# reedrosenbluth/LASS

Measured on AMD Instinct MI355X. Metric: clips/sec (10s@16kHz), higher is better.
Workload: dtype f32; 1 GPU; ResUNet30 separate() fp32, batch=16/GPU, 10s@16kHz clips, fixed precomputed condition embedding, seeded random-init weights (BASELINE configs[1]); samples_per_clip=160000, parallelism=clip-sharded x1

## Files before the change

### __graft_entry__.py

```python
import os
import subprocess
import sys

ROOT = os.path.dirname(os.path.abspath(__file__))
CSRC = os.path.join(ROOT, "lass_amd", "csrc")
LIB = os.path.join(CSRC, "liblass_hip.so")
SOURCES = ["api.hip", "conv.hip", "wino.hip", "wino4.hip", "pw_gemm.hip", "conv_bf16.hip", "conv_bf16_fused.hip", "stft.hip", "misc.hip", "text.hip", "audio_clap.hip", "resample.hip"]
FLAGS = ["-O3", "-std=c++17", "--offload-arch=gfx950", "-fPIC", "-fno-slp-vectorize"]
EXTRA_FLAGS = {}


def _hipcc() -> str:
    for c in (os.environ.get("HIPCC"), "/opt/rocm/bin/hipcc", "hipcc"):
        if c and (os.path.isabs(c) and os.path.exists(c) or not os.path.isabs(c)):
            return c
    return "hipcc"


STAMP = LIB + ".srchash"


def _src_hash() -> str:
    import hashlib

    h = hashlib.sha256()
    import glob

    h.update(repr((FLAGS, sorted(EXTRA_FLAGS.items()))).encode())

    deps = [os.path.join(CSRC, s) for s in SOURCES] + sorted(glob.glob(os.path.join(CSRC, "*.h"))) + [os.path.join(ROOT, "include", "lass_hip.h")]
    for d in deps:
        h.update(os.path.basename(d).encode())
        with open(d, "rb") as f:
            h.update(f.read())
    return h.hexdigest()


def _stale() -> bool:
    if not os.path.exists(LIB) or not os.path.exists(STAMP):
        return True
    with open(STAMP) as f:
        return f.read().strip() != _src_hash()


def build(force: bool = False) -> None:
    import fcntl

    if force or _stale():
        with open(os.path.join(CSRC, ".build.lock"), "w") as lock:
            fcntl.flock(lock, fcntl.LOCK_EX)
            if force or _stale():
                tmp = LIB + f".tmp{os.getpid()}"
                flags = FLAGS
                objs = [os.path.join(CSRC, f".{os.getpid()}.{s}.o") for s in SOURCES]
                print("[build]", _hipcc(), " ".join(flags), "-c", " ".join(SOURCES), "(parallel) && link", file=sys.stderr, flush=True)
                try:
                    procs = [subprocess.Popen([_hipcc()] + flags + EXTRA_FLAGS.get(s, []) + ["-c", s, "-o", o], cwd=CSRC)
                             for s, o in zip(SOURCES, objs)]
                    rcs = [pr.wait() for pr in procs]
                    if any(rcs):
# ... 54 lines not shown
```

### include/lass_hip.h

```cpp
#ifndef LASS_HIP_H
#define LASS_HIP_H

#include <stddef.h>
#include <stdint.h>

#ifdef __cplusplus
extern "C" {
#endif

typedef struct lass_ctx lass_ctx;

#define LASS_OK 0
#define LASS_ERR_ARG (-1)
#define LASS_ERR_HIP (-2)
#define LASS_ERR_STATE (-3)
#define LASS_ERR_WORKSPACE (-4)

#define LASS_F32 0
#define LASS_I64 1

#define LASS_COMPUTE_F32 0
#define LASS_COMPUTE_BF16 1
#define LASS_COMPUTE_BF16X3 2

int lass_version(void);

int lass_create(lass_ctx** out, int device_id);
int lass_create_multistft(lass_ctx** out, int device_id, int n_fft, int n_windows, const int* win_lengths,
                          int mask_window);
int lass_destroy(lass_ctx* ctx);

const char* lass_last_error(const lass_ctx* ctx);

int lass_set_param(lass_ctx* ctx, const char* name, const void* data, const int64_t* shape, int ndim, int dtype);

int lass_finalize(lass_ctx* ctx, int compute_mode);

int lass_workspace_bytes(const lass_ctx* ctx, int B, int L, size_t* bytes);

int lass_separate(lass_ctx* ctx, const float* mixture, const float* condition, float* out, int B, int L,
                  void* workspace, size_t workspace_bytes, void* stream);

int lass_graph_stats(const lass_ctx* ctx, long* captures, long* replays);
int lass_set_graph_replay(lass_ctx* ctx, int enabled);
int lass_set_wino4_splits(lass_ctx* ctx, int splits);

int lass_separate_components(lass_ctx* ctx, const float* const* mag, const float* cos_mask, const float* sin_mask,
                             const float* condition, float* out, int B, int L, void* workspace, size_t workspace_bytes,
                             void* stream);


int lass_stft_magphase(lass_ctx* ctx, const float* wav, int B, int L, float* mag, float* cos_out, float* sin_out,
                       float* real_out, float* imag_out, void* stream);

int lass_multi_stft(lass_ctx* ctx, const float* wav, int B, int L, int hop, int n_windows, const int* win_lengths,
                    float* const* mag, float* const* cos_out, float* const* sin_out, void* stream);

int lass_stft_components(lass_ctx* ctx, const float* wav, int B, int L, int n_fft, int hop, int n_windows,
                         const int* win_lengths, float* const* mag, float* const* cos_out, float* const* sin_out,
                         void* stream);

int lass_istft(lass_ctx* ctx, const float* real, const float* imag, int B, int T, int L, float* wav,
               float* frames_ws, void* stream);
int lass_istft_nfft(lass_ctx* ctx, const float* real, const float* imag, int B, int T, int L, int n_fft, int win_length,
                    float* wav, void* stream);

int lass_film(lass_ctx* ctx, const float* condition, int B, float* shift, void* stream);
int lass_film_width(const lass_ctx* ctx);
int lass_film_offset(const lass_ctx* ctx, const char* site);
int lass_film_raw(lass_ctx* ctx, const float* condition, int B, float* film, void* stream);

int lass_convblock(lass_ctx* ctx, const char* prefix, const float* x, int B, int H, int W, const float* shift,
                   float* y, float* scratch, void* stream);

int lass_encoder_block(lass_ctx* ctx, const char* name, const float* x, int B, int H, int W, const float* shift, float* y,
                       float* pool, float* scratch, void* stream);

int lass_front_end(lass_ctx* ctx, const float* wav, int B, int L, float* mag, float* cos_out, float* sin_out, float* x0,
                   void* stream);

int lass_workspace_tensor(const lass_ctx* ctx, int B, int L, const char* name, size_t* offset, int64_t shape[4],
                          int64_t strides[4]);

int lass_upconv(lass_ctx* ctx, const char* name, const float* x, int B, int h, int w, const float* shift, float* y,
                void* stream);

int lass_mask_apply(lass_ctx* ctx, const float* x12, const float* mag, const float* cos_in, const float* sin_in,
                    int B, int T, int Tpad, float* out_real, float* out_imag, void* stream);

int lass_sdr_stats(lass_ctx* ctx, const float* ref, const float* est, int B, int L, double* stats, void* stream);

int lass_mix_at_snr(lass_ctx* ctx, float* source, const float* noise, const float* snr_db, float* mixture, int B, int L,
                    double* scratch, void* stream);

#define LASS_WAV_PCM16 0
#define LASS_WAV_PCM32 1
#define LASS_WAV_F32 2
#define LASS_RESAMPLE_MAX_TAPS 16383
// ... 55 lines not shown
```

### lass_amd/_lib.py

```python
from __future__ import annotations

import ctypes
import os
from ctypes import POINTER, c_char_p, c_double, c_int, c_int64, c_long, c_size_t, c_void_p

_HERE = os.path.dirname(os.path.abspath(__file__))
LIB_PATH = os.environ.get("LASS_HIP_LIB") or os.path.join(_HERE, "csrc", "liblass_hip.so")

_lib = None

SYMBOLS = [
    ("lass_version", c_int, []),
    ("lass_create", c_int, [POINTER(c_void_p), c_int]),
    ("lass_create_multistft", c_int, [POINTER(c_void_p), c_int, c_int, c_int, POINTER(c_int), c_int]),
    ("lass_destroy", c_int, [c_void_p]),
    ("lass_last_error", c_char_p, [c_void_p]),
    ("lass_set_param", c_int, [c_void_p, c_char_p, c_void_p, POINTER(c_int64), c_int, c_int]),
    ("lass_finalize", c_int, [c_void_p, c_int]),
    ("lass_workspace_bytes", c_int, [c_void_p, c_int, c_int, POINTER(c_size_t)]),
    ("lass_separate", c_int, [c_void_p, c_void_p, c_void_p, c_void_p, c_int, c_int, c_void_p, c_size_t, c_void_p]),
    ("lass_stft_magphase", c_int, [c_void_p, c_void_p, c_int, c_int, c_void_p, c_void_p, c_void_p, c_void_p,
                                   c_void_p, c_void_p]),
    ("lass_mix_at_snr", c_int, [c_void_p, c_void_p, c_void_p, c_void_p, c_void_p, c_int, c_int, c_void_p, c_void_p]),
    ("lass_decode_resample", c_int, [c_void_p, c_void_p, c_int64, c_int, c_int, c_int, c_int, c_int, c_int, c_void_p, c_int,
                                     c_void_p, c_int, c_void_p]),
    ("lass_segment_mix", c_int, [c_void_p, c_void_p, c_int, c_int, c_void_p, c_void_p, c_int, c_void_p, c_void_p, c_void_p,
                                 c_void_p, c_void_p]),
    ("lass_multi_stft", c_int, [c_void_p, c_void_p, c_int, c_int, c_int, c_int, POINTER(c_int), POINTER(c_void_p),
                                POINTER(c_void_p), POINTER(c_void_p), c_void_p]),
    ("lass_graph_stats", c_int, [c_void_p, POINTER(c_long), POINTER(c_long)]),
    ("lass_set_graph_replay", c_int, [c_void_p, c_int]),
    ("lass_set_wino4_splits", c_int, [c_void_p, c_int]),
    ("lass_separate_components", c_int, [c_void_p, POINTER(c_void_p), c_void_p, c_void_p, c_void_p, c_void_p, c_int,
                                         c_int, c_void_p, c_size_t, c_void_p]),
    ("lass_stft_components", c_int, [c_void_p, c_void_p, c_int, c_int, c_int, c_int, c_int, POINTER(c_int),
                                     POINTER(c_void_p), POINTER(c_void_p), POINTER(c_void_p), c_void_p]),
    ("lass_istft_nfft", c_int, [c_void_p, c_void_p, c_void_p, c_int, c_int, c_int, c_int, c_int, c_void_p, c_void_p]),
    ("lass_istft", c_int, [c_void_p, c_void_p, c_void_p, c_int, c_int, c_int, c_void_p, c_void_p, c_void_p]),
    ("lass_film", c_int, [c_void_p, c_void_p, c_int, c_void_p, c_void_p]),
    ("lass_film_width", c_int, [c_void_p]),
    ("lass_film_offset", c_int, [c_void_p, c_char_p]),
    ("lass_film_raw", c_int, [c_void_p, c_void_p, c_int, c_void_p, c_void_p]),
    ("lass_convblock", c_int, [c_void_p, c_char_p, c_void_p, c_int, c_int, c_int, c_void_p, c_void_p, c_void_p,
                               c_void_p]),
    ("lass_encoder_block", c_int, [c_void_p, c_char_p, c_void_p, c_int, c_int, c_int, c_void_p, c_void_p, c_void_p,
                                   c_void_p, c_void_p]),
    ("lass_front_end", c_int, [c_void_p, c_void_p, c_int, c_int, c_void_p, c_void_p, c_void_p, c_void_p, c_void_p]),
    ("lass_workspace_tensor", c_int, [c_void_p, c_int, c_int, c_char_p, POINTER(c_size_t), POINTER(c_int64),
                                      POINTER(c_int64)]),
    ("lass_upconv", c_int, [c_void_p, c_char_p, c_void_p, c_int, c_int, c_int, c_void_p, c_void_p, c_void_p]),
    ("lass_mask_apply", c_int, [c_void_p, c_void_p, c_void_p, c_void_p, c_void_p, c_int, c_int, c_int, c_void_p,
                                c_void_p, c_void_p]),
    ("lass_sdr_stats", c_int, [c_void_p, c_void_p, c_void_p, c_int, c_int, c_void_p, c_void_p]),
    ("lass_text_create", c_int, [POINTER(c_void_p), c_int]),
    ("lass_text_destroy", c_int, [c_void_p]),
    ("lass_text_last_error", c_char_p, [c_void_p]),
    ("lass_text_set_param", c_int, [c_void_p, c_char_p, c_void_p, POINTER(c_int64), c_int]),
    ("lass_text_finalize", c_int, [c_void_p]),
    ("lass_text_layers", c_int, [c_void_p]),
    ("lass_text_workspace_bytes", c_int, [c_void_p, c_int, c_int, POINTER(c_size_t)]),
    ("lass_text_encode", c_int, [c_void_p, c_void_p, c_void_p, c_int, c_int, c_void_p, c_void_p, c_void_p, c_size_t,
                                 c_void_p]),
    ("lass_audioq_create", c_int, [POINTER(c_void_p), c_int]),
    ("lass_audioq_destroy", c_int, [c_void_p]),
    ("lass_audioq_last_error", c_char_p, [c_void_p]),
    ("lass_audioq_set_param", c_int, [c_void_p, c_char_p, c_void_p, POINTER(c_int64), c_int]),
    ("lass_audioq_finalize", c_int, [c_void_p]),
    ("lass_audioq_stages", c_int, [c_void_p]),
    ("lass_audioq_workspace_bytes", c_int, [c_void_p, c_int, POINTER(c_size_t)]),
    ("lass_audioq_encode_wave48k", c_int, [c_void_p, c_void_p, POINTER(c_int), c_int, c_int, c_void_p, c_void_p, c_void_p,
                                           c_size_t, c_void_p]),
    ("lass_audioq_encode_wave32k", c_int, [c_void_p, c_void_p, POINTER(c_int), c_int, c_int, c_void_p, c_void_p, c_void_p,
                                           c_size_t, c_void_p]),
    ("lass_set_profiling", c_int, [c_void_p, c_int]),
    ("lass_profile_count", c_int, [c_void_p]),
    ("lass_profile_get", c_int, [c_void_p, c_int, POINTER(c_char_p), POINTER(c_double), POINTER(c_int)]),
    ("lass_profile_reset", c_int, [c_void_p]),
]


class LassError(RuntimeError):
    pass


def load():
# ... 24 lines not shown
```

### lass_amd/csrc/api.hip

```cpp
#include <hip/hip_runtime.h>

#include <algorithm>
#include <cmath>
#include <cstdio>
#include <cstdlib>
#include <cstring>
#include <map>
#include <string>
#include <vector>

#include "../../include/lass_hip.h"
#include "kernels.h"

namespace {

struct EncSpec { const char* name; int cin, cout, dh, dw; };
struct DecSpec { const char* name; int cin, cout, uh, uw; };
const EncSpec kEnc[7] = {{"encoder_block1", 32, 32, 2, 2},   {"encoder_block2", 32, 64, 2, 2},
                         {"encoder_block3", 64, 128, 2, 2},  {"encoder_block4", 128, 256, 2, 2},
                         {"encoder_block5", 256, 384, 2, 2}, {"encoder_block6", 384, 384, 1, 2},
                         {"conv_block7a", 384, 384, 1, 1}};
const DecSpec kDec[6] = {{"decoder_block1", 384, 384, 1, 2}, {"decoder_block2", 384, 384, 2, 2},
                         {"decoder_block3", 384, 256, 2, 2}, {"decoder_block4", 256, 128, 2, 2},
                         {"decoder_block5", 128, 64, 2, 2},  {"decoder_block6", 64, 32, 2, 2}};
// ... 20 lines not shown
    int width = 0;
    int s1 = -1, s2 = -1;
    float *w1 = nullptr, *w2 = nullptr, *wsc = nullptr;
    float *u1 = nullptr, *u2 = nullptr, *usc = nullptr;
    float *u1f = nullptr, *u2f = nullptr;
    void *b1 = nullptr, *b2 = nullptr, *bsc16 = nullptr;
    void *b1l = nullptr, *b2l = nullptr, *bscl = nullptr;
    const float* bsc = nullptr;
};

struct ProfEntry {
    const char* name;
    double ms = 0;
    int launches = 0;
};

thread_local std::string g_create_err;

}

struct Geometry {
    int variant = 0;
    int nbr = 1;
    int wins[kMaxBranches] = {1024, 0, 0, 0};
    int nfft = 1024, nbins = 513, fcrop = 512;
    int mask_br = 0;
    int magphase_sem = 0;
};

struct lass_ctx {
    int device = 0;
    std::string err;
    Geometry g;
    EncSpec E[7];
    DecSpec D[6];
    int dec_cat[6] = {0};
    std::string pre_name[kMaxBranches];
    std::map<std::string, Raw> raw;
    bool finalized = false;
    float2* tw2k = nullptr;
    std::vector<Site> sites;
    std::map<std::string, int> site_idx;
    int n_shift = 0;
    float *film_W = nullptr, *film_b = nullptr, *bn_scale = nullptr, *bn_base = nullptr;
    float *bn0_s = nullptr, *bn0_h = nullptr;
    std::vector<ResBlock> enc, dec;
    int dec_site[6] = {0};
    void* up16[6] = {nullptr};
    void* up16l[6] = {nullptr};
    std::vector<void*> owned;
    int compute_mode = LASS_COMPUTE_F32;
    int wino4_mincin = 32;
    int ksplit_force = 0;
    float* stage_part = nullptr;
    size_t stage_part_floats = 0;
    bool fuse_catb = true;
    bool fuse_block = true;
    bool fuse_up = true;
    void* up_sc16 = nullptr;
    bool use_graph = true;
    struct GraphKey {
        const void *mix = nullptr, *cond = nullptr, *out = nullptr, *ws = nullptr;
        int B = 0, L = 0;
        unsigned long gen = 0;
        bool operator==(const GraphKey& o) const {
            return mix == o.mix && cond == o.cond && out == o.out && ws == o.ws && B == o.B && L == o.L && gen == o.gen;
        }
    };
    struct GraphEntry {
        GraphKey key;
        hipGraphExec_t exec = nullptr;
        size_t need = 0;
        int seen = 0;
        unsigned long used = 0;
        bool split = false;
    };
    std::map<std::pair<int, int>, bool> last_split;
    static constexpr int kGraphSlots = 4;
    GraphEntry g_slots[kGraphSlots];
    unsigned long g_tick = 0;
    std::vector<hipGraphExec_t> g_retired;
    hipStream_t g_stream = nullptr;
    int split_batch = 1;
    hipStream_t s2 = nullptr;
    hipEvent_t ev_fork = nullptr, ev_join = nullptr;
    unsigned long gen = 0;
    long g_replays = 0, g_captures = 0;
    bool profiling = false;
    std::vector<ProfEntry> prof;
    std::vector<hipEvent_t> ev_pool;
    struct Pending { int cls; hipEvent_t a, b; };
    std::vector<Pending> pending;
    size_t ev_used = 0;
};

namespace {

#define HIP_TRY(ctx, expr)                                                                                     \
    do {                                                                                                       \
        hipError_t _e = (expr);                                                                                \
        if (_e != hipSuccess) {                                                                                \
            (ctx)->err = std::string(#expr) + ": " + hipGetErrorString(_e);                                     \
            return LASS_ERR_HIP;                                                                               \
        }                                                                                                      \
    } while (0)

// ... 374 lines not shown
            return fail(c, LASS_ERR_STATE, "decoder_block6 with its transposed conv inside needs the fused bf16 kernel");
        ProfScope ps(c, st, P_CONV3X3);
        HIP_TRY(c, lass_launch_dec6u_fused_bf16(p, q, uq, st));
        return 0;
    }
    if (bf2 && !x0 && c->fuse_block && c->compute_mode == LASS_COMPUTE_BF16 && cat_in && f.head && rb.cin != rb.cout &&
        lass_dec6_fused_bf16_supported(p, q)) {
        ProfScope ps(c, st, P_CONV3X3);
        HIP_TRY(c, lass_launch_dec6_fused_bf16(p, q, st));
        return 0;
    }
    const bool sc_gemm = c->compute_mode == LASS_COMPUTE_F32 && !bf2 && rb.cin != rb.cout && !f.head && rb.cin >= kShortcutGemmMinCin &&
                         wino2 && q.w_wino4 && (ksplit > 0 || lass_wino4_supported(CONV2_SHORTCUT, q)) && lass_pw_gemm_supported(CONV2_SHORTCUT, q);
    if (sc_gemm) {
        const auto overlaps = [&](const float* a, long a_bs, long a_n, const float* b, long b_bs, long b_n) {
            return a < b + (size_t)(B - 1) * b_bs + b_n && b < a + (size_t)(B - 1) * a_bs + a_n;
        };
        if (overlaps(out, out_bs, rb.cout * HW, x, x_bs, rb.cin * HW) || overlaps(out, out_bs, rb.cout * HW, a2, rb.cout * HW, rb.cout * HW))
            return fail(c, LASS_ERR_STATE, "a block's output must not overlap its input or its intermediate");
        ProfScope ps(c, st, P_CONV3X3);
        HIP_TRY(c, lass_launch_pw_gemm(CONV2_SHORTCUT, q, st));
    }
    if (int r1 = launch_conv1()) return r1;
    ProfScope ps(c, st, P_CONV3X3);
    if (sc_gemm) {
        ConvArgs r = q;
        r.in2 = nullptr; r.in2_bs = 0; r.Cin2 = 0; r.w2 = nullptr; r.bias = nullptr;
        r.res = out; r.res_bs = out_bs;
        if (!lass_wino4_supported(CONV2_IDENT, r, sk)) return fail(c, LASS_ERR_STATE, "conv2 with the shortcut as residual");
        HIP_TRY(c, lass_launch_wino4(CONV2_IDENT, r, st, sk));
    } else if (rb.cin == rb.cout) {
        if (bf2)
            HIP_TRY(c, lass_launch_conv_bf16(k2, q, st));
        else if (wino2 && (x0 || ksplit > 0) && q.w_wino4 && lass_wino4_supported(k2, q, sk))
            HIP_TRY(c, lass_launch_wino4(k2, q, st, sk));
        else if (wino2)
            HIP_TRY(c, lass_launch_wino(k2, q, st));
        else
            HIP_TRY(c, lass_launch_conv(k2, q, st));
    } else {
        if (bf2)
            HIP_TRY(c, lass_launch_conv_bf16(CONV2_SHORTCUT, q, st));
        else if (wino2 && q.w_wino4 && lass_wino4_supported(CONV2_SHORTCUT, q))
            HIP_TRY(c, lass_launch_wino4(CONV2_SHORTCUT, q, st));
        else if (wino2)
            HIP_TRY(c, lass_launch_wino(CONV2_SHORTCUT, q, st));
        else
            HIP_TRY(c, lass_launch_conv(CONV2_SHORTCUT, q, st));
    }
    return 0;
}

constexpr int kTconvGemmMinCin = 128;

int run_upconv(lass_ctx* c, int di, const float* x, int B, int h, int w, const float* shift, float* out, long out_bs,
               hipStream_t st, const CatCopies* cb = nullptr, bool x_is_act_bf16 = false) {
    const DecSpec& d = c->D[di];
    const Site& s = c->sites[c->dec_site[di]];
    ConvArgs p;
    p.in = x; p.in_bs = (long)d.cin * h * w; p.Cin = d.cin;
    p.w = rawp(c, std::string("base.") + d.name + ".conv1.weight");
    p.N = p.Nw = d.cout * d.uh * d.uw;
    p.pro_scale = c->bn_scale + s.off; p.pro_shift = shift + s.off; p.pro_shift_bs = c->n_shift;
    p.out = out; p.out_bs = out_bs; p.B = B; p.H = h; p.W = w; p.up_h = d.uh;
    p.w_bf16 = c->up16[di]; p.w_bf16_lo = c->up16l[di];
    if (x_is_act_bf16) {
        if (c->compute_mode != LASS_COMPUTE_BF16 || !p.w_bf16 || !lass_bf16_supported(p))
            return fail(c, LASS_ERR_STATE, "activated bf16 input needs the bf16 kernels");
        p.in_bf16 = x;
    }
    if (cb) {
        if (c->compute_mode != LASS_COMPUTE_BF16 || !p.w_bf16 || !lass_bf16_supported(p))
            return fail(c, LASS_ERR_STATE, "blocked bf16 concat copies need the bf16 kernels");
        p.out = nullptr;
        p.out_bf16 = cb->raw; p.out_bf16_act = cb->act; p.out_oct0 = 0; p.out_noct = cb->noct;
        p.act_scale = cb->scale; p.act_shift = cb->shift; p.act_shift_bs = c->n_shift;
    }
    ProfScope ps(c, st, P_TCONV);
    if (c->compute_mode != LASS_COMPUTE_F32 && p.w_bf16 && lass_bf16_supported(p))
        HIP_TRY(c, lass_launch_conv_bf16(TCONV_ACT, p, st));
    else if (c->compute_mode == LASS_COMPUTE_F32 && d.cin >= kTconvGemmMinCin && lass_pw_gemm_supported(TCONV_ACT, p))
        HIP_TRY(c, lass_launch_pw_gemm(TCONV_ACT, p, st));
    else
        HIP_TRY(c, lass_launch_conv(TCONV_ACT, p, st));
    return 0;
}

struct Plan {
    int B, L, T, Tp;
    size_t total = 0;
    size_t mag, cosv, sinv, x0[kMaxBranches], shift, a2, cat[6], pool[6], center, decout[6], oreal, oimag;
    size_t kpart = 0;
    bool has_kpart = false;
    int eh[7], ew[7];
};

size_t bump(size_t& total, size_t floats) {
    const size_t off = total;
    total += (floats * sizeof(float) + 255) / 256 * 256;
    return off;
}

int make_plan(const lass_ctx* c, int B, int L, Plan* pl) {
    const Geometry& g = c->g;
    if (B <= 0 || L <= g.nfft / 2) return LASS_ERR_ARG;
    pl->B = B; pl->L = L;
    pl->T = 1 + L / LASS_HOP;
    pl->Tp = (pl->T + 31) / 32 * 32;
    const size_t clip_max = (size_t)c->dec_cat[5] * pl->Tp * g.fcrop * sizeof(float);
    if (clip_max > 0xFFFF0000ull) return LASS_ERR_ARG;
    size_t& t = pl->total;
    t = 0;
    const size_t spec = (size_t)B * pl->T * g.nbins;
    pl->mag = bump(t, spec); pl->cosv = bump(t, spec); pl->sinv = bump(t, spec);
    for (int k = 0; k < g.nbr; ++k) pl->x0[k] = bump(t, (size_t)B * pl->Tp * g.fcrop);
    pl->shift = bump(t, (size_t)B * c->n_shift);
    int h = pl->Tp, w = g.fcrop;
    size_t a2max = 0;
    for (int i = 0; i < 7; ++i) {
        pl->eh[i] = h; pl->ew[i] = w;
        const size_t o = (size_t)B * c->E[i].cout * h * w;
        if (o > a2max) a2max = o;
        h /= c->E[i].dh; w /= c->E[i].dw;
        if (i < 6) pl->pool[i] = bump(t, (size_t)B * c->E[i].cout * (i == 0 ? g.nbr : 1) * h * w);
    }
    pl->center = bump(t, (size_t)B * c->E[6].cout * pl->eh[6] * pl->ew[6]);
    for (int d = 0; d < 6; ++d) {
        const int e = 5 - d;
        const size_t hw = (size_t)pl->eh[e] * pl->ew[e];
        pl->cat[d] = bump(t, (size_t)B * c->dec_cat[d] * hw);
        pl->decout[d] = bump(t, (size_t)B * c->D[d].cout * hw);
    }
    pl->a2 = bump(t, a2max);
    pl->oreal = bump(t, spec); pl->oimag = bump(t, spec);
    size_t kmax = 0;
    for (int i = 1; i < 7; ++i) {
        const ResBlock& rb = trunk_block(c, i);
// ... 866 lines not shown
                if (r0) return r0;
                Plan pl0;
                if (!condition || !out || !workspace || make_plan(c, B, L, &pl0) || workspace_bytes < pl0.total ||
                    ((uintptr_t)workspace & 255) != 0)
                    return separate_any(c, mixture, condition, out, B, L, workspace, workspace_bytes, (hipStream_t)stream, false);
                slot->need = pl0.total;
                if (split_halves(c, B)) {
                    Plan ph0;
                    if (!make_plan(c, B / 2, L, &ph0) && 2 * ((ph0.total + 255) / 256 * 256) <= workspace_bytes)
                        slot->need = std::max(slot->need, 2 * ((ph0.total + 255) / 256 * 256));
                }
            }
            HIP_TRY(c, hipSetDevice(c->device));
            if (!c->g_stream) HIP_TRY(c, hipStreamCreateWithFlags(&c->g_stream, hipStreamNonBlocking));
            bool ok = false;
            if (hipStreamBeginCapture(c->g_stream, hipStreamCaptureModeThreadLocal) == hipSuccess) {
                const int r = separate_any(c, mixture, condition, out, B, L, workspace, workspace_bytes, c->g_stream, true);
                hipGraph_t graph = nullptr;
                const hipError_t e = hipStreamEndCapture(c->g_stream, &graph);
                if (r == 0 && e == hipSuccess && graph && hipGraphInstantiate(&slot->exec, graph, nullptr, nullptr, 0) == hipSuccess) {
                    ok = true;
                    if (auto it = c->last_split.find({B, L}); it != c->last_split.end()) slot->split = it->second;
                } else {
                    slot->exec = nullptr;
                }
                if (graph) (void)hipGraphDestroy(graph);
            }
            if (ok) {
                ++c->g_captures;
                HIP_TRY(c, hipGraphLaunch(slot->exec, (hipStream_t)stream));
                return 0;
            }
            (void)hipGetLastError();
            c->use_graph = false;
            c->err.clear();
        }
    }
    return separate_any(c, mixture, condition, out, B, L, workspace, workspace_bytes, (hipStream_t)stream, false);
}

int lass_set_graph_replay(lass_ctx* c, int enabled) {
    if (!c) return LASS_ERR_ARG;
    c->use_graph = enabled != 0;
    return 0;
}

int lass_set_wino4_splits(lass_ctx* c, int splits) {
    if (!c || (splits != 0 && splits != 1 && splits != 2 && splits != 4)) return fail(c, LASS_ERR_ARG, "lass_set_wino4_splits: 0, 1, 2 or 4");
    c->ksplit_force = splits;
    ++c->gen;
    return 0;
}

int lass_graph_stats(const lass_ctx* c, long* captures, long* replays) {
    if (!c) return LASS_ERR_ARG;
    if (captures) *captures = c->g_captures;
    if (replays) *replays = c->g_replays;
    return c->use_graph ? 1 : 0;
}

int lass_separate_components(lass_ctx* c, const float* const* mag, const float* cos_mask, const float* sin_mask,
                             const float* condition, float* out, int B, int L, void* workspace, size_t workspace_bytes,
                             void* stream) {
    if (!c) return LASS_ERR_ARG;
    if (!mag || !cos_mask || !sin_mask) return fail(c, LASS_ERR_ARG, "lass_separate_components: null pointer");
    Components comp;
    for (int k = 0; k < kMaxBranches; ++k) comp.mag[k] = k < c->g.nbr ? mag[k] : nullptr;
    comp.cosv = cos_mask; comp.sinv = sin_mask;
    return separate_impl(c, nullptr, &comp, condition, out, B, L, workspace, workspace_bytes, stream,
                         "lass_separate_components");
}

int lass_set_profiling(lass_ctx* c, int enabled) {
    if (!c) return LASS_ERR_ARG;
    if (enabled && c->ev_pool.size() < 2 * kProfPairs) {
        HIP_TRY(c, hipSetDevice(c->device));
        c->pending.reserve(kProfPairs);
        while (c->ev_pool.size() < 2 * kProfPairs) {
            hipEvent_t e;
            HIP_TRY(c, hipEventCreate(&e));
            c->ev_pool.push_back(e);
        }
    }
    c->profiling = enabled != 0;
    return 0;
}
int lass_profile_count(const lass_ctx* c) { return c ? P_COUNT : LASS_ERR_ARG; }
int lass_profile_get(lass_ctx* c, int i, const char** name, double* ms, int* launches) {
    if (!c || i < 0 || i >= P_COUNT) return LASS_ERR_ARG;
    prof_collect(c);
    if (name) *name = c->prof[i].name;
    if (ms) *ms = c->prof[i].ms;
    if (launches) *launches = c->prof[i].launches;
    return 0;
}
int lass_profile_reset(lass_ctx* c) {
    if (!c) return LASS_ERR_ARG;
    prof_collect(c);
    for (auto& p : c->prof) { p.ms = 0; p.launches = 0; }
    return 0;
}

}
```

### lass_amd/csrc/kernels.h

```cpp
#pragma once
#include <hip/hip_runtime.h>
#include <stddef.h>
#include <stdint.h>

constexpr int LASS_NFFT = 1024;
constexpr int LASS_HOP = 160;
constexpr int LASS_NBINS = 513;
constexpr int LASS_FCROP = 512;
constexpr int LASS_COND = 512;
constexpr int LASS_MAX_STFT_WINDOWS = 4;

struct ConvArgs {
    const float* in = nullptr;
    long in_bs = 0;
    int Cin = 0;
    const float* w = nullptr;
    int Nw = 0;
    const float* pro_scale = nullptr;
    const float* pro_shift = nullptr;
    int pro_shift_bs = 0;
    const float* in2 = nullptr;
    long in2_bs = 0;
    int Cin2 = 0;
    const float* w2 = nullptr;
// ... 22 lines not shown
    void* out_bf16_act = nullptr;
    const float* act_scale = nullptr;
    const float* act_shift = nullptr;
    int act_shift_bs = 0;
    int out_oct0 = 0;
    int out_noct = 0;
    const void* in2_bf16 = nullptr;
    void* pool_bf16 = nullptr;
    void* pool_bf16_act = nullptr;
    int pool_oct0 = 0;
    int pool_noct = 0;
    const float* pool_act_scale = nullptr;
    const float* pool_act_shift = nullptr;
    const float* pre_w = nullptr;
    const float* pre_b = nullptr;
    const float* mask_w = nullptr;
    const float* mask_b = nullptr;
    const float* mask_mag = nullptr;
    const float* mask_cos = nullptr;
    const float* mask_sin = nullptr;
    float* mask_re = nullptr;
    float* mask_im = nullptr;
    int mask_T = 0;
    int mask_nbins = LASS_NBINS;
    float* pool_out = nullptr;
    long pool_bs = 0;
    int pool_h = 2;
    int gx = 0, gy = 0;
    int xcd_map = 0;
};

inline bool lass_wino4_narrow(int H, int W) { return W % 32 == 16 && H % 32 == 0; }
struct Wino4Split {
    int n = 1;
    float* part = nullptr;
};

enum ConvKind { CONV1_ACT = 0, CONV2_IDENT = 1, CONV2_SHORTCUT = 2, TCONV_ACT = 3, CONV1_ACT_PRE = 4, CONV2_IDENT_PRE = 5 };

hipError_t lass_launch_conv(ConvKind kind, const ConvArgs& p, hipStream_t stream);

bool lass_wino_supported(const ConvArgs& p);
hipError_t lass_launch_wino(ConvKind kind, const ConvArgs& p, hipStream_t stream);
hipError_t lass_launch_wino_weights(const float* w, int Cout, int Cin, float* U, hipStream_t stream);
hipError_t lass_launch_wino_shortcut_weights(const float* w, int Cout, int Cin, float* U, hipStream_t stream);

bool lass_wino4_supported(ConvKind kind, const ConvArgs& p, const Wino4Split& sk = Wino4Split());
hipError_t lass_launch_wino4(ConvKind kind, const ConvArgs& p, hipStream_t stream, const Wino4Split& sk = Wino4Split());
hipError_t lass_launch_wino4_weights(const float* w, int Cout, int Cin, float* U, hipStream_t stream);

bool lass_pw_gemm_supported(ConvKind kind, const ConvArgs& p);
hipError_t lass_launch_pw_gemm(ConvKind kind, const ConvArgs& p, hipStream_t stream);

bool lass_bf16_supported(const ConvArgs& p);
hipError_t lass_launch_conv_bf16(ConvKind kind, const ConvArgs& p, hipStream_t stream);
hipError_t lass_launch_weights_bf16(const float* w, int Cout, int Cin, int taps, void* dst, int lo, int transposed,
                                    hipStream_t stream);

bool lass_enc1_fused_bf16_supported(const ConvArgs& p, const ConvArgs& q);
hipError_t lass_launch_enc1_fused_bf16(const ConvArgs& p, const ConvArgs& q, hipStream_t stream);
bool lass_dec6_fused_bf16_supported(const ConvArgs& p, const ConvArgs& q);
hipError_t lass_launch_dec6_fused_bf16(const ConvArgs& p, const ConvArgs& q, hipStream_t stream);

bool lass_dec6u_fused_bf16_supported(const ConvArgs& p, const ConvArgs& q, const ConvArgs& u);
hipError_t lass_launch_dec6u_fused_bf16(const ConvArgs& p, const ConvArgs& q, const ConvArgs& u, hipStream_t stream);
hipError_t lass_launch_compose_up_shortcut(const float* wsc, const float* wt, int Cin, int Cup, int Ccat, int Nsc, float* out,
                                           hipStream_t stream);

hipError_t lass_launch_multi_stft(const float* wav, int B, int L, int hop, int nwin, const int* n_fft,
                                  const float2* tw2k, float* const* mag, float* const* cosv, float* const* sinv,
                                  hipStream_t stream);
struct StftBranch {
    int wlen = 0;
    float *mag = nullptr, *cosv = nullptr, *sinv = nullptr, *real = nullptr, *imag = nullptr, *x0 = nullptr;
};
hipError_t lass_launch_stft2(const float* wav, int B, int L, int n_fft, int hop, int T, int Tpad, int nbr,
                             const StftBranch* br, int magphase_sem, const float* s0, const float* h0,
                             const float2* tw2k, hipStream_t stream);
hipError_t lass_launch_istft2(const float* real, const float* imag, int B, int T, int L, int n_fft, int wlen, int hop,
                              const float2* tw2k, float* wav, hipStream_t stream);

hipError_t lass_launch_film(const float* cond, int B, const float* Wf, const float* bf, const float* base, int n,
                            float* out, hipStream_t stream);
hipError_t lass_launch_pool(const float* in, long in_bs, int B, int C, int H, int W, int ph, int pw, float* out,
                            hipStream_t stream);
hipError_t lass_launch_mask(const float* x12, const float* wa, const float* ba, const float* mag, const float* cosv,
                            const float* sinv, int B, int T, int Tpad, int fcrop, float* out_real, float* out_imag,
                            hipStream_t stream);
hipError_t lass_launch_x0_from_mag(const float* mag, int B, int T, int Tpad, int fcrop, const float* s0,
                                   const float* h0, float* x0, hipStream_t stream);
hipError_t lass_launch_sdr(const float* ref, const float* est, int B, int L, double* stats, hipStream_t stream);
hipError_t lass_launch_mix_at_snr(float* source, const float* noise, const float* snr_db, float* mixture, int B, int L,
                                  double* ws, hipStream_t stream);
hipError_t lass_launch_segment_mix(const float* waveforms, int B, int L, const int* mix_num, const float* comp_db, int max_comp,
                                   const float* noise_db, float* mixture, float* segment, double* ws, hipStream_t stream);
hipError_t lass_launch_relayout_conv(const float* src, int Cout, int Cin, int taps, float* dst, hipStream_t stream);
hipError_t lass_launch_bnfold(const float* g, const float* beta, const float* mean, const float* var, int C, float eps,
                              float* scale, float* base, hipStream_t stream);

size_t lass_resample_table_floats(int up, int n_taps);
hipError_t lass_launch_decode_resample(const void* raw, long long row_stride, int B, int frames, int ch, int enc, int up, int down,
                                       const float* taps, int n_taps, float* out, int L_out, hipStream_t stream);
```

### lass_amd/engine.py

```python
from __future__ import annotations

from ctypes import byref, c_char_p, c_double, c_int, c_int64, c_size_t, c_void_p
from typing import Dict, Optional

import numpy as np
import torch

from . import _lib, arch


def _ptr(t: Optional[torch.Tensor]):
    return c_void_p(t.data_ptr()) if t is not None else c_void_p(0)


def _stream(device) -> c_void_p:
    return c_void_p(torch.cuda.current_stream(device).cuda_stream)


class Engine:

    def __init__(self, device="cuda:0", multistft=None):
        self.lib = _lib.load()
        self.device = torch.device(device)
        if self.device.type != "cuda":
# ... 297 lines not shown
            raise _lib.LassError(f"encoding must be one of {sorted(rs.ENCODINGS)}")
        B = raw_u8.shape[0]
        if raw_u8.shape[1] < int(frames) * int(channels) * rs.SAMPLE_BYTES[encoding]:
            raise _lib.LassError("raw_u8 rows are shorter than frames x channels samples")
        up, down = rs.ratio(rate_in, rate_out)
        L_out = rs.out_len(frames, up, down)
        fir = (up, down) != (1, 1)
        if fir and not rs.within_cap(up, down):
            raise _lib.LassError(f"resampling {rate_in} -> {rate_out} Hz needs {rs.n_taps(up, down)} taps, over the device "
                                 f"kernel's cap of {rs.MAX_TAPS}: resample on the host (wavio.read_wav)")
        taps = rs.device_taps(up, down, self.device) if fir else None
        if out is None:
            out = torch.empty(B, L_out, dtype=torch.float32, device=self.device)
        elif (tuple(out.shape) != (B, L_out) or out.dtype != torch.float32 or out.device != self.device
              or not out.is_contiguous()):
            raise _lib.LassError(f"out must be a contiguous float32 {(B, L_out)} tensor on {self.device}")
        stride = raw_u8.stride(0) if B > 1 else (raw_u8.shape[1] + 3) // 4 * 4
        rc = self.lib.lass_decode_resample(self.ctx, _ptr(raw_u8), stride, B, int(frames), int(channels), rs.ENCODINGS[encoding], up, down, _ptr(taps),
                                           taps.numel() if fir else 1, _ptr(out), L_out, _stream(self.device))
        _lib.check(self.ctx, rc, "lass_decode_resample")
        return out

    def resample(self, x: torch.Tensor, rate_in: int, rate_out: int) -> torch.Tensor:
        x = self._dev(x)
        one = x.dim() == 1
        x = x[None] if one else x
        y = self.decode_resample(x.view(torch.uint8), x.shape[1], 1, "f32", rate_in, rate_out)
        return y[0] if one else y

    def segment_mix(self, waveforms: torch.Tensor, mix_num: torch.Tensor, comp_db: torch.Tensor, noise_db: torch.Tensor):
        waveforms = self._dev(waveforms)
        B, L = waveforms.shape
        mix_num = mix_num.to(device=self.device, dtype=torch.int32).contiguous()
        comp_db = comp_db.to(device=self.device, dtype=torch.float32).contiguous()
        noise_db = noise_db.to(device=self.device, dtype=torch.float32).contiguous()
        if mix_num.shape != (B,) or noise_db.shape != (B,) or comp_db.dim() != 2 or comp_db.shape[0] != B:
            raise ValueError("segment_mix: mix_num (B), comp_db (B, max_mix_num - 1), noise_db (B) expected")
        mixture, segment = torch.empty_like(waveforms), torch.empty_like(waveforms)
        scratch = torch.empty(B, 4, dtype=torch.float64, device=self.device)
        rc = self.lib.lass_segment_mix(self.ctx, _ptr(waveforms), B, L, _ptr(mix_num), _ptr(comp_db), int(comp_db.shape[1]),
                                       _ptr(noise_db), _ptr(mixture), _ptr(segment), _ptr(scratch), _stream(self.device))
        _lib.check(self.ctx, rc, "lass_segment_mix")
        return mixture, segment

    def graph_stats(self):
        from ctypes import c_long
        cap, rep = c_long(), c_long()
        on = self.lib.lass_graph_stats(self.ctx, byref(cap), byref(rep))
        return bool(on), cap.value, rep.value

    def set_graph_replay(self, on: bool):
        _lib.check(self.ctx, self.lib.lass_set_graph_replay(self.ctx, 1 if on else 0), "lass_set_graph_replay")

    def set_profiling(self, on: bool):
        self.lib.lass_set_profiling(self.ctx, 1 if on else 0)

    def profile(self, reset: bool = True) -> Dict[str, tuple]:
        out = {}
        for i in range(self.lib.lass_profile_count(self.ctx)):
            name, ms, n = c_char_p(), c_double(), c_int()
            self.lib.lass_profile_get(self.ctx, i, byref(name), byref(ms), byref(n))
            out[name.value.decode()] = (ms.value, n.value)
        if reset:
            self.lib.lass_profile_reset(self.ctx)
        return out


def arch_cond() -> int:
    return 512


_ENGINES: Dict[int, Engine] = {}


def get_engine(device) -> Engine:
    device = torch.device(device)
    idx = device.index if device.index is not None else torch.cuda.current_device()
    if idx not in _ENGINES:
        _ENGINES[idx] = Engine(torch.device("cuda", idx))
    return _ENGINES[idx]
```

Measured before the change: 1040 clips/s.

## Add persistent streaming MFMA kernel for small-Cin transposed convolutions

Adds a persistent-workgroup fp32 MFMA kernel for decoder transposed convolutions with Cin 64 or 128. The weights stay resident in LDS, the fused BN+leaky prologue is applied while staging input chunks, and global loads of the next chunk and next tile are software-pipelined. It is routed by default in f32 mode ahead of the previous pw_gemm and direct paths. The cost is extra LDS pressure and a grid tied to the CU count, which may limit occupancy.

```diff
diff --git a/__graft_entry__.py b/__graft_entry__.py
--- a/__graft_entry__.py
+++ b/__graft_entry__.py
@@ -5,7 +5,7 @@
 ROOT = os.path.dirname(os.path.abspath(__file__))
 CSRC = os.path.join(ROOT, "lass_amd", "csrc")
 LIB = os.path.join(CSRC, "liblass_hip.so")
-SOURCES = ["api.hip", "conv.hip", "wino.hip", "wino4.hip", "pw_gemm.hip", "conv_bf16.hip", "conv_bf16_fused.hip", "stft.hip", "misc.hip", "text.hip", "audio_clap.hip", "resample.hip"]
+SOURCES = ["api.hip", "conv.hip", "wino.hip", "wino4.hip", "pw_gemm.hip", "tconv_stream.hip", "conv_bf16.hip", "conv_bf16_fused.hip", "stft.hip", "misc.hip", "text.hip", "audio_clap.hip", "resample.hip"]
 FLAGS = ["-O3", "-std=c++17", "--offload-arch=gfx950", "-fPIC", "-fno-slp-vectorize"]
 EXTRA_FLAGS = {}
 
diff --git a/include/lass_hip.h b/include/lass_hip.h
--- a/include/lass_hip.h
+++ b/include/lass_hip.h
@@ -44,6 +44,9 @@
 int lass_graph_stats(const lass_ctx* ctx, long* captures, long* replays);
 int lass_set_graph_replay(lass_ctx* ctx, int enabled);
 int lass_set_wino4_splits(lass_ctx* ctx, int splits);
+int lass_set_tconv_stream(lass_ctx* ctx, int on);
+int lass_tconv_stream_workgroups(lass_ctx* ctx, const char* name, const float* x, int B, int h, int w, const float* shift,
+                                 float* y);
 
 int lass_separate_components(lass_ctx* ctx, const float* const* mag, const float* cos_mask, const float* sin_mask,
                              const float* condition, float* out, int B, int L, void* workspace, size_t workspace_bytes,
diff --git a/lass_amd/_lib.py b/lass_amd/_lib.py
--- a/lass_amd/_lib.py
+++ b/lass_amd/_lib.py
@@ -31,6 +31,8 @@
     ("lass_graph_stats", c_int, [c_void_p, POINTER(c_long), POINTER(c_long)]),
     ("lass_set_graph_replay", c_int, [c_void_p, c_int]),
     ("lass_set_wino4_splits", c_int, [c_void_p, c_int]),
+    ("lass_set_tconv_stream", c_int, [c_void_p, c_int]),
+    ("lass_tconv_stream_workgroups", c_int, [c_void_p, c_char_p, c_void_p, c_int, c_int, c_int, c_void_p, c_void_p]),
     ("lass_separate_components", c_int, [c_void_p, POINTER(c_void_p), c_void_p, c_void_p, c_void_p, c_void_p, c_int,
                                          c_int, c_void_p, c_size_t, c_void_p]),
     ("lass_stft_components", c_int, [c_void_p, c_void_p, c_int, c_int, c_int, c_int, c_int, POINTER(c_int),
diff --git a/lass_amd/csrc/api.hip b/lass_amd/csrc/api.hip
--- a/lass_amd/csrc/api.hip
+++ b/lass_amd/csrc/api.hip
@@ -96,6 +96,7 @@
     int compute_mode = LASS_COMPUTE_F32;
     int wino4_mincin = 32;
     int ksplit_force = 0;
+    bool tconv_stream = true;
     float* stage_part = nullptr;
     size_t stage_part_floats = 0;
     bool fuse_catb = true;
@@ -576,9 +577,18 @@
 }
 
 constexpr int kTconvGemmMinCin = 128;
-
-int run_upconv(lass_ctx* c, int di, const float* x, int B, int h, int w, const float* shift, float* out, long out_bs,
-               hipStream_t st, const CatCopies* cb = nullptr, bool x_is_act_bf16 = false) {
+constexpr int kTconvStreamMaxCin = 128;
+
+enum TconvRoute { TCONV_BF16, TCONV_STREAM, TCONV_GEMM, TCONV_DIRECT };
+
+TconvRoute tconv_route(const lass_ctx* c, const DecSpec& d, const ConvArgs& p) {
+    if (c->compute_mode != LASS_COMPUTE_F32) return p.w_bf16 && lass_bf16_supported(p) ? TCONV_BF16 : TCONV_DIRECT;
+    if (c->tconv_stream && d.cin <= kTconvStreamMaxCin && lass_tconv_stream_supported(p)) return TCONV_STREAM;
+    if (d.cin >= kTconvGemmMinCin && lass_pw_gemm_supported(TCONV_ACT, p)) return TCONV_GEMM;
+    return TCONV_DIRECT;
+}
+
+ConvArgs upconv_args(const lass_ctx* c, int di, const float* x, int B, int h, int w, const float* shift, float* out, long out_bs) {
     const DecSpec& d = c->D[di];
     const Site& s = c->sites[c->dec_site[di]];
     ConvArgs p;
@@ -588,6 +598,13 @@
     p.pro_scale = c->bn_scale + s.off; p.pro_shift = shift + s.off; p.pro_shift_bs = c->n_shift;
     p.out = out; p.out_bs = out_bs; p.B = B; p.H = h; p.W = w; p.up_h = d.uh;
     p.w_bf16 = c->up16[di]; p.w_bf16_lo = c->up16l[di];
+    return p;
+}
+
+int run_upconv(lass_ctx* c, int di, const float* x, int B, int h, int w, const float* shift, float* out, long out_bs,
+               hipStream_t st, const CatCopies* cb = nullptr, bool x_is_act_bf16 = false) {
+    const DecSpec& d = c->D[di];
+    ConvArgs p = upconv_args(c, di, x, B, h, w, shift, out, out_bs);
     if (x_is_act_bf16) {
         if (c->compute_mode != LASS_COMPUTE_BF16 || !p.w_bf16 || !lass_bf16_supported(p))
             return fail(c, LASS_ERR_STATE, "activated bf16 input needs the bf16 kernels");
@@ -601,12 +618,12 @@
         p.act_scale = cb->scale; p.act_shift = cb->shift; p.act_shift_bs = c->n_shift;
     }
     ProfScope ps(c, st, P_TCONV);
-    if (c->compute_mode != LASS_COMPUTE_F32 && p.w_bf16 && lass_bf16_supported(p))
-        HIP_TRY(c, lass_launch_conv_bf16(TCONV_ACT, p, st));
-    else if (c->compute_mode == LASS_COMPUTE_F32 && d.cin >= kTconvGemmMinCin && lass_pw_gemm_supported(TCONV_ACT, p))
-        HIP_TRY(c, lass_launch_pw_gemm(TCONV_ACT, p, st));
-    else
-        HIP_TRY(c, lass_launch_conv(TCONV_ACT, p, st));
+    switch (tconv_route(c, d, p)) {
+        case TCONV_BF16: HIP_TRY(c, lass_launch_conv_bf16(TCONV_ACT, p, st)); break;
+        case TCONV_STREAM: HIP_TRY(c, lass_launch_tconv_stream(p, st)); break;
+        case TCONV_GEMM: HIP_TRY(c, lass_launch_pw_gemm(TCONV_ACT, p, st)); break;
+        case TCONV_DIRECT: HIP_TRY(c, lass_launch_conv(TCONV_ACT, p, st)); break;
+    }
     return 0;
 }
 
@@ -1579,6 +1596,25 @@
     return 0;
 }
 
+int lass_set_tconv_stream(lass_ctx* c, int on) {
+    if (!c) return LASS_ERR_ARG;
+    c->tconv_stream = on != 0;
+    ++c->gen;
+    return 0;
+}
+
+int lass_tconv_stream_workgroups(lass_ctx* c, const char* name, const float* x, int B, int h, int w, const float* shift, float* y) {
+    int r = check_ready(c);
+    if (r) return -1;
+    if (!name || !x || !shift || !y) return -1;
+    for (int i = 0; i < 6; ++i)
+        if (std::string("base.") + c->D[i].name == name) {
+            const ConvArgs p = upconv_args(c, i, x, B, h, w, shift, y, (long)c->D[i].cout * h * c->D[i].uh * w * c->D[i].uw);
+            return tconv_route(c, c->D[i], p) == TCONV_STREAM ? lass_tconv_stream_grid(p) : 0;
+        }
+    return -1;
+}
+
 int lass_graph_stats(const lass_ctx* c, long* captures, long* replays) {
     if (!c) return LASS_ERR_ARG;
     if (captures) *captures = c->g_captures;
diff --git a/lass_amd/csrc/kernels.h b/lass_amd/csrc/kernels.h
--- a/lass_amd/csrc/kernels.h
+++ b/lass_amd/csrc/kernels.h
@@ -98,6 +98,10 @@
 bool lass_pw_gemm_supported(ConvKind kind, const ConvArgs& p);
 hipError_t lass_launch_pw_gemm(ConvKind kind, const ConvArgs& p, hipStream_t stream);
 
+bool lass_tconv_stream_supported(const ConvArgs& p);
+int lass_tconv_stream_grid(const ConvArgs& p);
+hipError_t lass_launch_tconv_stream(const ConvArgs& p, hipStream_t stream);
+
 bool lass_bf16_supported(const ConvArgs& p);
 hipError_t lass_launch_conv_bf16(ConvKind kind, const ConvArgs& p, hipStream_t stream);
 hipError_t lass_launch_weights_bf16(const float* w, int Cout, int Cin, int taps, void* dst, int lo, int transposed,
diff --git a/lass_amd/csrc/tconv_stream.hip b/lass_amd/csrc/tconv_stream.hip
--- /dev/null
+++ b/lass_amd/csrc/tconv_stream.hip
@@ -0,0 +1,182 @@
+#include <hip/hip_runtime.h>
+#include <limits.h>
+#include <algorithm>
+#include "kernels.h"
+#include "pixel_ops.h"
+
+namespace {
+
+constexpr int NTHREADS = 256;
+constexpr int PB = 128;
+constexpr int KC = 16;
+
+typedef float f32x16 __attribute__((ext_vector_type(16)));
+
+template <int NCH, int TN>
+__global__ __launch_bounds__(NTHREADS, TN == 2 ? 3 : 1) void tconv_stream_kernel(ConvArgs p, int items, int tiles) {
+    constexpr int K = NCH * KC, N = TN * 64;
+    static_assert(NCH >= 4 && NCH % 2 == 0 && K <= NTHREADS, "chunk pipeline: two stages, three chunks of look-ahead");
+    __shared__ __attribute__((aligned(16))) float lds[K * N + 2 * KC * PB + 3 * NTHREADS];
+    float* const wres = lds;
+    float* const xbuf = lds + K * N;
+    float* const sct = xbuf + 2 * KC * PB;
+    float* const sht = sct + NTHREADS;
+    const int tid = threadIdx.x, lane = tid & 63, wave = tid >> 6;
+    const int wn = wave >> 1, wp = wave & 1;
+    const unsigned P = (unsigned)p.H * (unsigned)p.W;
+    const int G = (int)gridDim.x;
+
+    const int kr = tid >> 5, c4 = (tid & 31) * 4;
+    const auto xptr = [&](int it) {
+        const int b = it / tiles, t = it - b * tiles;
+        return p.in + (size_t)b * p.in_bs + min((unsigned)t * PB + (unsigned)c4, P - 4u) + (size_t)kr * P;
+    };
+    const auto hptr = [&](int it) { return p.pro_shift + (size_t)(it / tiles) * p.pro_shift_bs + tid % K; };
+    struct Stage {
+        float4 x0, x1;
+    };
+    Stage S0, S1;
+    const auto gload = [&](Stage& st, const float* xs, int ch) {
+        st.x0 = *reinterpret_cast<const float4*>(xs + (size_t)(ch * KC) * P);
+        st.x1 = *reinterpret_cast<const float4*>(xs + (size_t)(ch * KC + 8) * P);
+    };
+    const auto act = [](float4 v, float s, float h) {
+        return make_float4(leaky(fmaf(v.x, s, h)), leaky(fmaf(v.y, s, h)), leaky(fmaf(v.z, s, h)), leaky(fmaf(v.w, s, h)));
+    };
+    const auto sstore = [&](const Stage& st, int buf, int par, int ch) {
+        const int k = ch * KC + kr;
+        const float s0 = sct[k], s1 = sct[k + 8], h0 = sht[par * NTHREADS + k], h1 = sht[par * NTHREADS + k + 8];
+        float* lb = xbuf + buf * (KC * PB) + kr * PB + c4;
+        *reinterpret_cast<float4*>(lb) = act(st.x0, s0, h0);
+        *reinterpret_cast<float4*>(lb + 8 * PB) = act(st.x1, s1, h1);
+    };
+
+    int it = (int)blockIdx.x;
+    const float* xs = xptr(it);
+    gload(S0, xs, 0);
+    gload(S1, xs, 1);
+    const float hfirst = *hptr(it);
+    for (int i0 = tid; i0 < K * N / 4; i0 += 8 * NTHREADS) {
+        float4 t[8];
+#pragma unroll
+        for (int j = 0; j < 8; ++j) t[j] = reinterpret_cast<const float4*>(p.w)[i0 + j * NTHREADS];
+#pragma unroll
+        for (int j = 0; j < 8; ++j) reinterpret_cast<float4*>(wres)[i0 + j * NTHREADS] = t[j];
+    }
+    sct[tid] = p.pro_scale[tid % K];
+    sht[tid] = hfirst;
+    __syncthreads();
+    sstore(S0, 0, 0, 0);
+    gload(S0, xs, 2);
+    __syncthreads();
+
+    const int foa = (lane >> 5) * N + (lane & 31) + wn * (TN * 32);
+    const int fob = (lane >> 5) * PB + (lane & 31) + wp * 64;
+    f32x16 acc[TN][2];
+    const auto mma = [&](int buf, int ch) {
+        const float* la = wres + ch * (KC * N) + foa;
+        const float* lb = xbuf + buf * (KC * PB) + fob;
+        float fa[KC / 2][TN], fb[KC / 2][2];
+#pragma unroll
+        for (int ks = 0; ks < KC / 2; ++ks) {
+#pragma unroll
+            for (int i = 0; i < TN; ++i) fa[ks][i] = la[2 * ks * N + 32 * i];
+            fb[ks][0] = lb[2 * ks * PB];
+            fb[ks][1] = lb[2 * ks * PB + 32];
+        }
+        __builtin_amdgcn_sched_barrier(0);
+#pragma unroll
+        for (int ks = 0; ks < KC / 2; ++ks)
+#pragma unroll
+            for (int i = 0; i < TN; ++i) {
+                acc[i][0] = __builtin_amdgcn_mfma_f32_32x32x2f32(fa[ks][i], fb[ks][0], acc[i][0], 0, 0, 0);
+                acc[i][1] = __builtin_amdgcn_mfma_f32_32x32x2f32(fa[ks][i], fb[ks][1], acc[i][1], 0, 0, 0);
+            }
+        __builtin_amdgcn_sched_barrier(0);
+    };
+
+    for (int par = 0; it < items; it += G, par ^= 1) {
+        const int nit = min(it + G, items - 1);
+        const float* xn = xptr(nit);
+        const float hn = *hptr(nit);
+#pragma unroll
+        for (int i = 0; i < TN; ++i)
+#pragma unroll
+            for (int r = 0; r < 16; ++r) acc[i][0][r] = acc[i][1][r] = 0.f;
+#pragma unroll
+        for (int ch = 0; ch < NCH; ++ch) {
+            mma(ch & 1, ch);
+            const int c1 = ch + 1, c3 = ch + 3;
+            if (ch & 1) {
+                sstore(S0, 0, c1 < NCH ? par : par ^ 1, c1 % NCH);
+                gload(S0, c3 < NCH ? xs : xn, c3 % NCH);
+            } else {
+                sstore(S1, 1, par, c1);
+                gload(S1, c3 < NCH ? xs : xn, c3 % NCH);
+            }
+            if (ch == NCH - 2) sht[(par ^ 1) * NTHREADS + tid] = hn;
+            __syncthreads();
+        }
+
+        const int b = it / tiles;
+        const unsigned p0 = (unsigned)(it - b * tiles) * PB;
+#pragma unroll
+        for (int tp = 0; tp < 2; ++tp) {
+            const unsigned pj = p0 + (unsigned)(wp * 64 + tp * 32 + (lane & 31));
+            if (pj >= P) continue;
+            const unsigned y = pj / (unsigned)p.W, x = pj - y * (unsigned)p.W;
+            const int uhw = p.up_h * 2;
+            const size_t oHW = (size_t)P * uhw;
+            const unsigned oW = 2u * (unsigned)p.W;
+            const size_t s2 = uhw == 4 ? (size_t)oW : oHW, s4 = (size_t)(8 / uhw) * oHW;
+            float* ob = p.out + (size_t)b * p.out_bs + (size_t)(y * p.up_h) * oW + 2u * x;
+#pragma unroll
+            for (int tn = 0; tn < TN; ++tn) {
+                const int nb = wn * (TN * 32) + tn * 32 + 4 * (lane >> 5);
+                float* o = ob + (size_t)(nb / uhw) * oHW;
+#pragma unroll
+                for (int r = 0; r < 16; r += 2)
+                    *reinterpret_cast<float2*>(o + (r >> 2) * s4 + ((r & 2) >> 1) * s2) = make_float2(acc[tn][tp][r], acc[tn][tp][r + 1]);
+            }
+        }
+        xs = xn;
+    }
+}
+
+int cu_count() {
+    static int n = 0;
+    if (n == 0) {
+        int dev = 0, v = 0;
+        if (hipGetDevice(&dev) == hipSuccess && hipDeviceGetAttribute(&v, hipDeviceAttributeMultiprocessorCount, dev) == hipSuccess && v > 0)
+            n = v;
+        else
+            return 256;
+    }
+    return n;
+}
+
+}
+
+bool lass_tconv_stream_supported(const ConvArgs& p) {
+    if (!lass_pw_gemm_supported(TCONV_ACT, p) || p.N != p.Nw || p.pro_shift_bs < p.Cin) return false;
+    if (!((p.Cin == 64 && p.N == 128) || (p.Cin == 128 && p.N == 256))) return false;
+    const long tiles = ((long)p.H * p.W + PB - 1) / PB;
+    return tiles * p.B <= INT_MAX;
+}
+
+int lass_tconv_stream_grid(const ConvArgs& p) {
+    const long items = (((long)p.H * p.W + PB - 1) / PB) * p.B;
+    return (int)std::min(items, (long)(p.Cin == 64 ? 3 : 1) * cu_count());
+}
+
+hipError_t lass_launch_tconv_stream(const ConvArgs& p, hipStream_t stream) {
+    if (!lass_tconv_stream_supported(p)) return hipErrorInvalidValue;
+    const int tiles = (int)(((long)p.H * p.W + PB - 1) / PB);
+    const int items = tiles * p.B;
+    const dim3 grid((unsigned)lass_tconv_stream_grid(p));
+    if (p.Cin == 64)
+        hipLaunchKernelGGL((tconv_stream_kernel<4, 2>), grid, dim3(NTHREADS), 0, stream, p, items, tiles);
+    else
+        hipLaunchKernelGGL((tconv_stream_kernel<8, 4>), grid, dim3(NTHREADS), 0, stream, p, items, tiles);
+    return hipGetLastError();
+}
diff --git a/lass_amd/engine.py b/lass_amd/engine.py
--- a/lass_amd/engine.py
+++ b/lass_amd/engine.py
@@ -373,6 +373,18 @@
     def set_graph_replay(self, on: bool):
         _lib.check(self.ctx, self.lib.lass_set_graph_replay(self.ctx, 1 if on else 0), "lass_set_graph_replay")
 
+    def set_tconv_stream(self, on: bool):
+        _lib.check(self.ctx, self.lib.lass_set_tconv_stream(self.ctx, 1 if on else 0), "lass_set_tconv_stream")
+
+    def tconv_stream_workgroups(self, name: str, x: torch.Tensor, shift: torch.Tensor, cout: int, up) -> int:
+        x = self._dev(x)
+        B, _cin, h, w = x.shape
+        y = torch.empty(B, cout, h * up[0], w * up[1], dtype=torch.float32, device=self.device)
+        n = self.lib.lass_tconv_stream_workgroups(self.ctx, name.encode(), _ptr(x), B, h, w, _ptr(shift), _ptr(y))
+        if n < 0:
+            raise _lib.LassError("lass_tconv_stream_workgroups: bad argument")
+        return n
+
     def set_profiling(self, on: bool):
         self.lib.lass_set_profiling(self.ctx, 1 if on else 0)
 
```

Result: no change. 1045 clips/s, median of 4 (+0.5%).
